# ishine/minimax-speech

Hardware: AMD Instinct MI355X
Metric: 24 kHz audio-seconds generated per wall-second per node (CosyVoice2-0.5B-shaped LM + flow + DAC-VAE, end to end) (higher is better)
Workload: dtype bf16

## Files before the change

### minimax-speech_amd/csrc/fused.hip

```cpp
#include "common.h"
#include "../../include/mmx_hip.h"
#include <type_traits>

namespace {

typedef __attribute__((ext_vector_type(4))) unsigned int u32x4_t;

__device__ unsigned long long* g_tail_stamps = nullptr;
#define TSTAMP(i) do { if constexpr (LAB) { if (st && lane == 0) st[(i)] = __builtin_amdgcn_s_memtime(); } } while (0)

template <typename T> struct FT;
template <> struct FT<bf16_t> { static constexpr int E = 8, KB = 32; typedef short8_t frag_t; };
template <> struct FT<float> { static constexpr int E = 4, KB = 16; typedef float4_t frag_t; };

template <typename T>
__device__ __forceinline__ float4_t mma(typename FT<T>::frag_t a, typename FT<T>::frag_t b, float4_t c) {
    if constexpr (sizeof(T) == 2) {
        return __builtin_amdgcn_mfma_f32_16x16x32_bf16(a, b, c, 0, 0, 0);
    } else {
#pragma unroll
        for (int s = 0; s < 4; ++s) c = __builtin_amdgcn_mfma_f32_16x16x4f32(a[s], b[s], c, 0, 0, 0);
        return c;
    }
}

__host__ __device__ constexpr int tile_pitch(int K, int esz) { return ((K * esz + 255) & ~255) + 32; }

template <typename T, int NF, int PF_>
struct WRing {
    static constexpr int E = FT<T>::E, PF = PF_;
    u32x4_t w[PF][NF];
    __device__ __forceinline__ void prime(const T* wb, long ns, int nk, int nf) {
#pragma unroll
        for (int p = 0; p < PF; ++p)
#pragma unroll
            for (int j = 0; j < NF; ++j)
                w[p][j] = *reinterpret_cast<const u32x4_t*>(wb + (j < nf ? j : 0) * ns + (long)(p < nk ? p : nk - 1) * 64 * E);
    }
};

template <typename T, int MF, int NF, int PF, int NS = 1, int RW = 4>
__device__ __forceinline__ void stage_run(WRing<T, RW, PF>& ring, const char* a_lane, int pitch, int cin_steps,
                                          const T* wb, long ns, int nk, const T* wbn, long nsn, int nkn, int nfn,
                                          float4_t (&acc)[MF][NF], int plane = 0, int tap_pitch = 0) {
    constexpr int E = FT<T>::E, KB = FT<T>::KB;
    typedef typename FT<T>::frag_t frag_t;
    if (tap_pitch == 0) tap_pitch = pitch;
    constexpr int AD = (PF % 2) ? PF : ((MF == 1 && PF >= 4) ? 4 : 2);
    static_assert(PF % AD == 0, "ring depths");
    if constexpr (NS == 2 && MF == 4) {
        frag_t a2[2][MF];
        int rt = 0, rc = 0, rs = 0, rp = 0;
        auto read_u = [&](frag_t (&dst)[MF]) {
            const char* ap = a_lane + rt * tap_pitch + rc * (KB * (int)sizeof(T)) + rp * plane;
#pragma unroll
            for (int i = 0; i < MF; ++i) dst[i] = *reinterpret_cast<const frag_t*>(ap + i * 16 * pitch);
            if (rp == 0) rp = 1;
            else {
                rp = 0;
                if (rs + 1 < nk) {
                    ++rs;
                    if (++rc == cin_steps) { rc = 0; ++rt; }
                }
            }
        };
        auto group2 = [&](int ks, auto last_c) {
            constexpr bool LAST = decltype(last_c)::value;
#pragma unroll
            for (int p = 0; p < PF; ++p) {
                frag_t b[NF];
#pragma unroll
                for (int jj = 0; jj < NF; ++jj) b[jj] = __builtin_bit_cast(frag_t, ring.w[p][jj]);
                if constexpr (LAST) {
                    if (wbn) {
                        const T* src = wbn + (long)(p < nkn ? p : nkn - 1) * 64 * E;
#pragma unroll
                        for (int jj = 0; jj < RW; ++jj) ring.w[p][jj] = *reinterpret_cast<const u32x4_t*>(src + (jj < nfn ? jj : 0) * nsn);
                    }
                } else {
                    const T* src = wb + (long)(ks + p + PF) * 64 * E;
#pragma unroll
                    for (int jj = 0; jj < NF; ++jj) ring.w[p][jj] = *reinterpret_cast<const u32x4_t*>(src + jj * ns);
                }
#pragma unroll
                for (int s2 = 0; s2 < 2; ++s2) {
                    read_u(a2[(s2 + 1) & 1]);
                    __builtin_amdgcn_sched_barrier(0);
#pragma unroll
                    for (int i = 0; i < MF; ++i)
#pragma unroll
                        for (int jj = 0; jj < NF; ++jj) acc[i][jj] = mma<T>(a2[s2][i], b[jj], acc[i][jj]);
                    __builtin_amdgcn_sched_barrier(0);
                }
            }
        };
        read_u(a2[0]);
        for (int ks = 0; ks + PF < nk; ks += PF) group2(ks, std::false_type{});
        group2(nk - PF, std::true_type{});
        return;
    }
    frag_t a[AD][NS][MF];
    int rt = 0, rc = 0, rs = 0;
    auto read_a = [&](frag_t (&dst)[NS][MF]) {
        const char* ap = a_lane + rt * tap_pitch + rc * (KB * (int)sizeof(T));
#pragma unroll
        for (int s2 = 0; s2 < NS; ++s2)
#pragma unroll
            for (int i = 0; i < MF; ++i) dst[s2][i] = *reinterpret_cast<const frag_t*>(ap + s2 * plane + i * 16 * pitch);
        if (rs + 1 < nk) {
            ++rs;
            if (++rc == cin_steps) { rc = 0; ++rt; }
        }
    };
    auto group = [&](int ks, auto last_c) {
        constexpr bool LAST = decltype(last_c)::value;
#pragma unroll
        for (int p = 0; p < PF; ++p) {
            read_a(a[(p + AD - 1) % AD]);
            frag_t b[NF];
#pragma unroll
            for (int jj = 0; jj < NF; ++jj) b[jj] = __builtin_bit_cast(frag_t, ring.w[p][jj]);
            if constexpr (LAST) {
                if (wbn) {
                    const T* src = wbn + (long)(p < nkn ? p : nkn - 1) * 64 * E;
#pragma unroll
                    for (int jj = 0; jj < RW; ++jj) ring.w[p][jj] = *reinterpret_cast<const u32x4_t*>(src + (jj < nfn ? jj : 0) * nsn);
                }
            } else {
                const T* src = wb + (long)(ks + p + PF) * 64 * E;
#pragma unroll
                for (int jj = 0; jj < NF; ++jj) ring.w[p][jj] = *reinterpret_cast<const u32x4_t*>(src + jj * ns);
            }
            __builtin_amdgcn_sched_barrier(0);
#pragma unroll
            for (int s2 = 0; s2 < NS; ++s2)
#pragma unroll
                for (int i = 0; i < MF; ++i)
#pragma unroll
                    for (int jj = 0; jj < NF; ++jj) acc[i][jj] = mma<T>(a[p % AD][s2][i], b[jj], acc[i][jj]);
            __builtin_amdgcn_sched_barrier(0);
        }
    };
#pragma unroll
    for (int s_ = 0; s_ < AD - 1; ++s_) read_a(a[s_]);
    for (int ks = 0; ks + PF < nk; ks += PF) group(ks, std::false_type{});
    group(nk - PF, std::true_type{});
}

template <typename T, int MF, int NF, int PF, int NS, int RW, bool WP>
__device__ __forceinline__ void stage_run_w(WRing<T, RW, PF>& ring, const char* a_lane, int pitch, int cin_steps,
                                            const T* wb, long ns, int nk, long wlo, const T* wbn, long nsn, int nkn, int nfn,
                                            float4_t (&acc)[MF][NF], int plane = 0, int tap_pitch = 0) {
    if constexpr (!WP) {
        stage_run<T, MF, NF, PF, NS, RW>(ring, a_lane, pitch, cin_steps, wb, ns, nk, wbn, nsn, nkn, nfn, acc, plane, tap_pitch);
    } else {
        stage_run<T, MF, NF, PF, NS, RW>(ring, a_lane, pitch, cin_steps, wb, ns, nk, wb + wlo, ns, nk, NF, acc, plane, tap_pitch);
        stage_run<T, MF, NF, PF, 1, RW>(ring, a_lane, pitch, cin_steps, wb + wlo, ns, nk, wbn, nsn, nkn, nfn, acc, 0, tap_pitch);
    }
}

template <int MF, int NF>
__device__ __forceinline__ void zero_acc(float4_t (&acc)[MF][NF]) {
#pragma unroll
    for (int i = 0; i < MF; ++i)
#pragma unroll
        for (int j = 0; j < NF; ++j) acc[i][j] = float4_t{0.f, 0.f, 0.f, 0.f};
}

constexpr int PATCH_FLOATS = 16 * 68;
constexpr int TAIL_PRM_FLOATS = 6 * 256 + 1024;
template <int NF>
__device__ __forceinline__ void to_rows(const float4_t (&acc)[NF], float* patch, int lane, float (&v)[NF * 4]) {
    constexpr int LDC = NF * 16 + 4;
    const int g = lane >> 4, l16 = lane & 15;
#pragma unroll
    for (int j = 0; j < NF; ++j)
#pragma unroll
        for (int r = 0; r < 4; ++r) patch[(4 * g + r) * LDC + j * 16 + l16] = acc[j][r];
    __builtin_amdgcn_fence(__ATOMIC_RELEASE, "wavefront");
    __builtin_amdgcn_wave_barrier();
    const float* src = patch + (lane >> 2) * LDC + (lane & 3) * (NF * 4);
#pragma unroll
    for (int c = 0; c < NF * 4; c += 4) {
        const float4_t t = *reinterpret_cast<const float4_t*>(src + c);
        v[c] = t[0]; v[c + 1] = t[1]; v[c + 2] = t[2]; v[c + 3] = t[3];
    }
    __builtin_amdgcn_wave_barrier();
}

constexpr int SPATCH_FLOATS = 16 * 20;
__device__ __forceinline__ void to_rows_sp(const float4_t (&acc)[2], float* patch, int lane, float (&v)[8]) {
    constexpr int LDC = 20;
    const int g = lane >> 4, l16 = lane & 15;
    const float* src = patch + (lane >> 2) * LDC + (lane & 1) * 8;
#pragma unroll
    for (int j = 0; j < 2; ++j) {
#pragma unroll
        for (int r = 0; r < 4; ++r) patch[(4 * g + r) * LDC + l16] = acc[j][r];
        __builtin_amdgcn_fence(__ATOMIC_RELEASE, "wavefront");
        __builtin_amdgcn_wave_barrier();
        if (((lane >> 1) & 1) == j) {
            const float4_t t0 = *reinterpret_cast<const float4_t*>(src), t1 = *reinterpret_cast<const float4_t*>(src + 4);
            v[0] = t0[0]; v[1] = t0[1]; v[2] = t0[2]; v[3] = t0[3];
            v[4] = t1[0]; v[5] = t1[1]; v[6] = t1[2]; v[7] = t1[3];
        }
        __builtin_amdgcn_wave_barrier();
    }
}
template <int NF, bool SP>
__device__ __forceinline__ void rows_of(const float4_t (&acc)[NF], float* patch, int lane, float (&v)[NF * 4]) {
// ... 495 lines not shown
        __syncthreads();
        TSTAMP(HK ? sb + 2 : 14 + ch * 12);
        const T* wn = ch + 1 < NCH ? w1_pass((ch + 1) * PPC) : (p.next.wqkv ? qkv_pass<T, NW, PW>(p.next.wqkv, wave, lane, 0) : nullptr);
        if constexpr (WP && !HK) {
            constexpr int NKQ = NK2 / 2;
            const T* wh = w2_w + (long)(ch * NK2) * 64 * E;
            stage_run_w<T, MF, NFN, PF, NS, PW, WP>(ring, buf0 + l16 * P0 + g * 16, P0, NKQ, wh, ns2, NKQ, (long)C * CF, wh + (long)NKQ * 64 * E, ns2, NKQ, NFN, acc2, PL0);
            stage_run_w<T, MF, NFN, PF, NS, PW, WP>(ring, buf0 + NKQ * KB * (int)sizeof(T) + l16 * P0 + g * 16, P0, NKQ, wh + (long)NKQ * 64 * E, ns2, NKQ, (long)C * CF, wn, ns1, NK1, PW, acc2, PL0);
        } else
        stage_run_w<T, MF, NFN, PF, NS, PW, WP>(ring, buf0 + l16 * P0 + g * 16, P0, NK2, w2_w + (long)(ch * NK2) * 64 * E, ns2, NK2, (long)C * CF, wn, ns1, NK1, PW, acc2, PL0);
        TSTAMP(HK ? sb + 3 : 15 + ch * 12);
        __syncthreads();
        TSTAMP(HK ? sb + 4 : 16 + ch * 12);
    }
    float* wpatch = HK ? reinterpret_cast<float*>(buf0) + wave * PATCH_FLOATS : patch;
    {
        float* xw = p.x + (long)b * p.x_bs;
        float b2[CW];
        loadn<CW>(prm + PRM_B2 + col0, b2);
#pragma unroll
        for (int i = 0; i < MF; ++i) {
            float v[CW];
            to_rows<NFN>(acc2[i], wpatch, lane, v);
            const int t = t0 + i * 16 + rl;
#pragma unroll
            for (int c = 0; c < CW; ++c) x1[i][c] = (x1[i][c] + v[c] + b2[c]) * rm[i];
            if (t < Tn) {
                storen<CW>(xw + (long)t * C + col0, x1[i]);
                if (p.act_out)
                    storen_T<TI, CW>(reinterpret_cast<TI*>(p.act_out) + (long)b * p.act_bs + (long)t * p.act_ld + col0, x1[i]);
            }
        }
    }
    TSTAMP(31);
    if (p.next.wqkv) {
        float n1g[CW], n1b[CW];
        loadn<CW>(prm + PRM_N1G + col0, n1g);
        loadn<CW>(prm + PRM_N1B + col0, n1b);
        ln_qkv<T, MF, PF, NW, NS, PW, WP>(x1, n1g, n1b, p.next, p.eps, a1, wpatch, stats, ring, b, t0, Tn, wave, lane, PL1, st);
    }
    TSTAMP(63);
}

template <typename T, int BM, int PF, int NW, int NS = 1, int OCC = 1, int PW = 4, bool WP = false>
__global__ __launch_bounds__(64 * NW, OCC) void est_tail_kernel(MmxEstTailParams p) {
    est_tail_tile<T, BM, PF, NW, NS, PW, WP>(p, blockIdx.x);
}

template <typename T, int BM, int PF, int NW, int NS = 1, bool WP = false>
__global__ __launch_bounds__(64 * NW) void est_resnet_kernel(MmxEstResnetParams p) {
    constexpr int MF = BM / 16, MH = MF + 1, E = FT<T>::E, KB = FT<T>::KB, C = 256;
    constexpr int WC = C / NW, CW = WC / 4, NFN = WC / 16;
    constexpr int P1 = tile_pitch(C, sizeof(T));
    constexpr int PLH = (BM + 16) * P1;
    constexpr bool PRECISE = sizeof(T) == 4;
    extern __shared__ __attribute__((aligned(16))) char smem[];
    const int cin = p.cin;
    const int PA = tile_pitch(cin, sizeof(T));
    const int PLA = (BM + 18) * PA;
    char* ain = smem;
    char* h1 = ain + NS * PLA;
    float* patch_all = reinterpret_cast<float*>(h1 + NS * PLH);
    float* stats = patch_all + NW * PATCH_FLOATS;
    const int tid = threadIdx.x, lane = tid & 63, wave = tid >> 6;
    const int g = lane >> 4, l16 = lane & 15, rl = lane >> 2;
    float* patch = patch_all + wave * PATCH_FLOATS;
    const int b = blockIdx.y, t0 = p.t_begin + blockIdx.x * BM, Tn = p.T;
    const int col0 = wave * WC + (lane & 3) * CW;
    const int cs = cin / KB;
    const T* w1 = reinterpret_cast<const T*>(p.w1) + (long)lane * E;
    const T* w2 = reinterpret_cast<const T*>(p.w2) + (long)lane * E;
    const T* wr = reinterpret_cast<const T*>(p.wr) + (long)lane * E;
    const int nk1 = 3 * cs, nk2 = 3 * (C / KB), nkr = cs;
    const long ns1 = (long)nk1 * 64 * E, ns2 = (long)nk2 * 64 * E, nsr = (long)nkr * 64 * E;
    const T* w1_w = w1 + (long)(wave * NFN) * ns1;
    const T* w2_w = w2 + (long)(wave * NFN) * ns2;
    const T* wr_w = wr + (long)(wave * NFN) * nsr;
    WRing<T, 4, PF> ring;
    ring.prime(w1_w, ns1, nk1, NFN);
    const float* rmk = p.rowmask ? p.rowmask + (long)b * p.rm_bs : nullptr;
    float bb[CW], tv[CW], gg[CW], be[CW], rm1[MH];
    loadn<CW>(p.b1 + col0, bb);
    loadn<CW>(p.tv + (long)b * p.tv_bs + col0, tv);
    loadn<CW>(p.g1 + col0, gg);
    loadn<CW>(p.be1 + col0, be);
#pragma unroll
    for (int i = 0; i < MH; ++i) {
        const int t = t0 - 16 + i * 16 + rl;
        rm1[i] = (t >= 0 && t < Tn) ? (rmk ? rmk[t] : 1.f) : 0.f;
    }
    if constexpr (NS == 1) load_tile<T>(reinterpret_cast<const T*>(p.a_in) + (long)b * p.a_bs, p.lda, t0 - 18, Tn, BM + 18, cin, ain, PA, tid, 64 * NW);
    else load_tile_split(reinterpret_cast<const float*>(p.a_in) + (long)b * p.a_bs, p.lda, t0 - 18, Tn, BM + 18, cin, ain, PA, PLA, tid, 64 * NW);
    __syncthreads();

    {
        float4_t acc[MH][NFN];
        zero_acc(acc);
        stage_run_w<T, MH, NFN, PF, NS, 4, WP>(ring, ain + l16 * PA + g * 16, PA, cs, w1_w, ns1, nk1, (long)C * 3 * cin, w2_w, ns2, nk2, NFN, acc, PLA);
        float hv[MH][CW];
#pragma unroll
        for (int i = 0; i < MH; ++i) {
            to_rows<NFN>(acc[i], patch, lane, hv[i]);
#pragma unroll
            for (int c = 0; c < CW; ++c) hv[i][c] += bb[c];
        }
        layernorm_rows<MH, CW, NW>(hv, stats, gg, be, p.eps, wave, lane);
#pragma unroll
        for (int i = 0; i < MH; ++i) {
            const int t = t0 - 16 + i * 16 + rl;
            float o[CW];
#pragma unroll
            for (int c = 0; c < CW; ++c) {
                const float y = act_c<ACT_MISH, PRECISE>(hv[i][c], 0.f) * rm1[i];
                o[c] = t >= 0 ? (y + tv[c]) * rm1[i] : 0.f;
            }
            store_tile<T, NS, CW>(h1 + (i * 16 + rl) * P1 + col0 * (int)sizeof(T), PLH, o);
        }
    }
    float br[CW];
    loadn<CW>(p.b2 + col0, bb);
    loadn<CW>(p.g2 + col0, gg);
    loadn<CW>(p.be2 + col0, be);
    loadn<CW>(p.br + col0, br);
    __syncthreads();
    float h2[MF][CW];
    {
        float4_t acc[MF][NFN];
        zero_acc(acc);
        stage_run_w<T, MF, NFN, PF, NS, 4, WP>(ring, h1 + (14 + l16) * P1 + g * 16, P1, C / KB, w2_w, ns2, nk2, (long)C * 3 * C, wr_w, nsr, nkr, NFN, acc, PLH);
#pragma unroll
        for (int i = 0; i < MF; ++i) {
            to_rows<NFN>(acc[i], patch, lane, h2[i]);
#pragma unroll
            for (int c = 0; c < CW; ++c) h2[i][c] += bb[c];
        }
        layernorm_rows<MF, CW, NW>(h2, stats, gg, be, p.eps, wave, lane);
#pragma unroll
        for (int i = 0; i < MF; ++i)
#pragma unroll
            for (int c = 0; c < CW; ++c) h2[i][c] = act_c<ACT_MISH, PRECISE>(h2[i][c], 0.f) * rm1[i + 1];
    }
    {
        if (p.next.wqkv) { loadn<CW>(p.next.n1g + col0, gg); loadn<CW>(p.next.n1b + col0, be); }
        float4_t acc[MF][NFN];
        zero_acc(acc);
        const T* wq0 = p.next.wqkv ? qkv_pass<T, NW>(p.next.wqkv, wave, lane, 0) : nullptr;
        stage_run_w<T, MF, NFN, PF, NS, 4, WP>(ring, ain + (18 + l16) * PA + g * 16, PA, cs, wr_w, nsr, nkr, (long)C * cin, wq0, (long)(C / KB) * 64 * E, C / KB, 4, acc, PLA);
        float* xw = p.x + (long)b * p.x_bs;
#pragma unroll
        for (int i = 0; i < MF; ++i) {
            float v[CW];
            to_rows<NFN>(acc[i], patch, lane, v);
            const int t = t0 + i * 16 + rl;
#pragma unroll
            for (int c = 0; c < CW; ++c) h2[i][c] += v[c] + br[c];
            if (t < Tn) storen<CW>(xw + (long)t * C + col0, h2[i]);
        }
    }
    __syncthreads();
    if (p.next.wqkv) ln_qkv<T, MF, PF, NW, NS, 4, WP>(h2, gg, be, p.next, p.eps, h1, patch, stats, ring, b, t0, Tn, wave, lane, PLH);
}


__host__ __device__ constexpr int dac_pitch(int cp) { return (((cp * 2 + 31) / 32) | 1) * 32; }
constexpr int DAC_PATCH_FLOATS = 16 * 52;

template <int C, int BM, int WR, int WC, int NS, int PF, bool WP = false>
__global__ __launch_bounds__(256) void dac_ru_kernel(MmxDacRuParams p) {
    typedef bf16_t T;
    constexpr int E = 8, KB = 32, NF = 3, CP = (C + 31) / 32 * 32, PA = dac_pitch(CP);
    constexpr int BMW = BM / WR, MF = BMW / 16;
    constexpr int NK7 = 7 * CP / KB, NK1 = CP / KB;
    constexpr bool PRECISE = NS > 1;
    static_assert(WR * WC == 4 && WC * NF * 16 == C && NK7 % PF == 0 && NK1 % PF == 0, "wave grid / ring depth");
    typedef std::conditional_t<NS == 1, bf16_t, float> TA;
    extern __shared__ __attribute__((aligned(16))) char smem[];
    const int d = p.dil, halo = 3 * d, rows_in = BM + 2 * halo;
    const int PLA = rows_in * PA, PLM = BM * PA;
    char* ain = smem;
    char* mid = ain + NS * PLA;
    float* patch_all = reinterpret_cast<float*>(mid + NS * PLM);
    float* prm = patch_all + 4 * DAC_PATCH_FLOATS;
    auto snk = [](float x, float alpha, float inv) {
        const float sn = PRECISE ? sin_cw(alpha * x) : __sinf(alpha * x);
        return x + inv * (sn * sn);
    };
    const int tid = threadIdx.x, lane = tid & 63, wave = tid >> 6;
    const int g = lane >> 4, l16 = lane & 15, rl = lane >> 2;
    const int wr = wave / WC, wc = wave % WC;
    float* patch = patch_all + wave * DAC_PATCH_FLOATS;
    const int b = blockIdx.y, t0 = blockIdx.x * BM;
    const int len = p.lens ? p.lens[b] : p.T;
    const int lc = len > 0 ? len : 1;
    const float* xb = p.x + (long)b * p.x_bs;

    const T* w7 = reinterpret_cast<const T*>(p.w7) + (long)lane * E;
    const T* w1 = reinterpret_cast<const T*>(p.w1) + (long)lane * E;
    const long ns7 = (long)NK7 * 64 * E, ns1 = (long)NK1 * 64 * E;
    const T* w7_w = w7 + (long)(wc * NF) * ns7;
    const T* w1_w = w1 + (long)(wc * NF) * ns1;
    WRing<T, NF, PF> ring;
    ring.prime(w7_w, ns7, NK7, NF);

    for (int id = tid; id < 8 * CP; id += 256) {
        const int v = id / CP, c = id - v * CP;
        const float* src = v == 0 ? p.a0 : v == 1 ? p.a2 : v == 2 ? p.b7 : v == 3 ? p.b1 : v == 4 ? p.alpha_next : v == 5 ? p.a0 : v == 6 ? p.a2 : p.alpha_next;
        const float val = (c < C && src) ? src[c] : 0.f;
        prm[id] = v < 5 ? val : 1.0f / (val + 1e-9f);
    }
    __syncthreads();
    {
        constexpr int CPR = CP / 4, U = 16;
// ... 98 lines not shown
        loadn<12>(prm + 4 * CP + col, an);
        loadn<12>(prm + 7 * CP + col, in);
        float* xo = p.x_out + (long)b * p.x_bs;
#pragma unroll
        for (int i = 0; i < MF; ++i) {
            float v[12];
            to_rows<NF>(acc[i], patch, lane, v);
            const int t = t0 + wr * BMW + i * 16 + rl;
            const bool live = t < len;
#pragma unroll
            for (int c = 0; c < 12; ++c) {
                float y = v[c] + b1[c];
                y = y > 0.f ? y : y * p.slope;
                v[c] = live ? y + xr[i][c] : 0.f;
            }
            if (t < p.T) {
                storen<12>(xo + (long)t * C + col, v);
                if (p.act_out) {
#pragma unroll
                    for (int c = 0; c < 12; ++c) v[c] = snk(v[c], an[c], in[c]);
                    TA* ao = reinterpret_cast<TA*>(p.act_out) + (long)b * p.x_bs + (long)t * C + col;
                    if constexpr (NS == 1) {
                        uint2 h0, h1, h2;
                        h0.x = pack_bf16x2(v[0], v[1]); h0.y = pack_bf16x2(v[2], v[3]);
                        h1.x = pack_bf16x2(v[4], v[5]); h1.y = pack_bf16x2(v[6], v[7]);
                        h2.x = pack_bf16x2(v[8], v[9]); h2.y = pack_bf16x2(v[10], v[11]);
                        *reinterpret_cast<uint2*>(ao) = h0;
                        *reinterpret_cast<uint2*>(ao + 4) = h1;
                        *reinterpret_cast<uint2*>(ao + 8) = h2;
                    } else {
                        storen<12>(reinterpret_cast<float*>(ao), v);
                    }
                }
            }
        }
    }
}

template <int C, int BM, int NS>
size_t dac_ru_lds(int dil) {
    constexpr int CP = (C + 31) / 32 * 32, PA = dac_pitch(CP);
    return (size_t)NS * ((size_t)(BM + 6 * dil) * PA + (size_t)BM * PA) + 4 * DAC_PATCH_FLOATS * 4 + 8 * CP * 4;
}

template <typename T, int BM, int NW, int NS = 1>
size_t tail_lds() {
    if (NS == 2 && BM == 64 && sizeof(T) == 2)
        return (size_t)NS * 2 * BM * tile_pitch(256, sizeof(T)) + (size_t)NW * SPATCH_FLOATS * 4 + (size_t)BM * NW * 4 + (size_t)TAIL_PRM_FLOATS * 4;
    return NS * ((size_t)BM * tile_pitch(512, sizeof(T)) + (size_t)BM * tile_pitch(256, sizeof(T))) + (size_t)NW * PATCH_FLOATS * 4 + (size_t)BM * NW * 4 +
           (size_t)TAIL_PRM_FLOATS * 4;
}
template <typename T, int BM, int NW, int NS = 1>
size_t resnet_lds(int cin) {
    return NS * ((size_t)(BM + 18) * tile_pitch(cin, sizeof(T)) + (size_t)(BM + 16) * tile_pitch(256, sizeof(T))) + (size_t)NW * PATCH_FLOATS * 4 +
           (size_t)(BM + 16) * NW * 4;
}

int check_next(const MmxEstNext& nx, int dtype, int T_) {
    if (!nx.wqkv) return MMX_OK;
    MMX_CHECK_ARG(nx.n1g && nx.n1b && nx.q_out);
    MMX_CHECK_ARG(((uintptr_t)nx.q_out % 16) == 0 && nx.q_bs % 8 == 0);
    if (dtype == MMX_X2) {
        if (nx.vt_out) {
            MMX_CHECK_ARG(nx.ldq % 8 == 0 && nx.ldq >= 2048 && nx.q_bs % 8 == 0 && nx.ldvt % 8 == 0 && nx.ldvt >= ((T_ + 7) / 8) * 8);
            MMX_CHECK_ARG(((uintptr_t)nx.vt_out % 16) == 0 && nx.vt_bs % 8 == 0 && nx.vt_bs >= 2 * 512 * (int64_t)nx.ldvt);
        } else {
            MMX_CHECK_ARG(nx.ldq % 4 == 0 && nx.ldq >= 1536 && nx.q_bs % 4 == 0);
        }
    } else if (dtype == MMX_BF16) {
        MMX_CHECK_ARG(nx.vt_out && nx.ldq % 8 == 0 && nx.ldq >= 1024 && nx.ldvt % 8 == 0 && nx.ldvt >= ((T_ + 7) / 8) * 8);
        MMX_CHECK_ARG(((uintptr_t)nx.vt_out % 16) == 0 && nx.vt_bs % 8 == 0);
    } else {
        MMX_CHECK_ARG(nx.ldq % 4 == 0 && nx.ldq >= 1536);
    }
    return MMX_OK;
}

}

#if MMX_LAB
extern "C" int mmx_lab_tail_stamps(void* buf) {
    unsigned long long* p = reinterpret_cast<unsigned long long*>(buf);
    const hipError_t e = hipMemcpyToSymbol(HIP_SYMBOL(g_tail_stamps), &p, sizeof(p));
    return e == hipSuccess ? MMX_OK : -(int)e - 1000;
}
#endif

extern "C" int mmx_est_tail(const MmxEstTailParams* pp, int dtype, int bm, int cfg, hipStream_t stream) {
    MMX_CHECK_ARG(pp != nullptr);
    const MmxEstTailParams& p = *pp;
    const bool wplanes = dtype == MMX_X2W;
    if (wplanes) dtype = MMX_X2;
    MMX_CHECK_ARG(p.ao && p.x && p.wo && p.w1 && p.w2 && p.bo && p.b1 && p.b2 && p.n3g && p.n3b && p.B > 0 && p.T > 0);
    MMX_CHECK_ARG(p.t_begin >= 0 && p.t_begin < p.T && p.t_begin % 16 == 0);
    MMX_CHECK_ARG(p.ldao >= 512 && p.ldao % (dtype == MMX_X2 ? 4 : 8) == 0 && p.ao_bs % (dtype == MMX_X2 ? 4 : 8) == 0 && p.x_bs % 4 == 0);
    MMX_CHECK_ARG(((uintptr_t)p.ao % 16) == 0 && ((uintptr_t)p.x % 16) == 0);
    MMX_CHECK_ARG(!p.act_out || (p.act_ld % (dtype == MMX_X2 ? 4 : 8) == 0 && p.act_bs % (dtype == MMX_X2 ? 4 : 8) == 0 && ((uintptr_t)p.act_out % 16) == 0));
    if (int rc = check_next(p.next, dtype, p.T)) return rc;
    const int nw = (cfg >> 4) & 15, occ2 = (cfg >> 8) & 1;
#define TAILT(TT, BM, PF, NW, NS, OCC, PW, ...)                                                           \
    do {                                                                                                   \
        const size_t lds = tail_lds<TT, BM, NW, NS>();                                                     \
        MMX_CHECK_ARG(lds * OCC <= 160 * 1024);                                                            \
        MMX_LDS_OPT_IN((est_tail_kernel<TT, BM, PF, NW, NS, OCC, PW __VA_OPT__(,) __VA_ARGS__>), lds);     \
        hipLaunchKernelGGL((est_tail_kernel<TT, BM, PF, NW, NS, OCC, PW __VA_OPT__(,) __VA_ARGS__>), dim3((p.T - p.t_begin + BM - 1) / BM, p.B), dim3(64 * NW), lds, stream, p); \
    } while (0)
// ... 40 lines not shown
        } else return MMX_EARG;
    } else if (dtype == MMX_F32) {
        if (bm == 32 && (nw == 0 || nw == 4)) TAIL(float, 32, 4, 4);
        else if (bm == 16 && (nw == 0 || nw == 4)) TAIL(float, 16, 8, 4);
        else return MMX_EARG;
    } else return MMX_EARG;
#undef TAIL
#undef TAILN
#undef TAILO
#undef TAILP
#undef TAILT
    MMX_LAUNCH_CHECK();
    return MMX_OK;
}

extern "C" int mmx_est_resnet(const MmxEstResnetParams* pp, int dtype, int bm, int cfg, hipStream_t stream) {
    MMX_CHECK_ARG(pp != nullptr);
    const MmxEstResnetParams& p = *pp;
    const bool wplanes = dtype == MMX_X2W;
    if (wplanes) dtype = MMX_X2;
    MMX_CHECK_ARG(p.a_in && p.x && p.w1 && p.w2 && p.wr && p.b1 && p.b2 && p.br && p.g1 && p.be1 && p.g2 && p.be2 && p.tv);
    MMX_CHECK_ARG(p.t_begin >= 0 && p.t_begin < p.T && p.t_begin % 16 == 0);
    MMX_CHECK_ARG(p.B > 0 && p.T > 0 && p.cin >= 64 && p.cin % 32 == 0 && p.cin <= 512 && p.lda >= p.cin);
    MMX_CHECK_ARG(p.lda % (dtype == MMX_X2 ? 4 : 8) == 0 && p.a_bs % (dtype == MMX_X2 ? 4 : 8) == 0);
    MMX_CHECK_ARG(((uintptr_t)p.a_in % 16) == 0 && ((uintptr_t)p.x % 16) == 0 && p.x_bs % 4 == 0 && p.tv_bs % 4 == 0 && ((uintptr_t)p.tv % 16) == 0);
    if (int rc = check_next(p.next, dtype, p.T)) return rc;
    const int pf_req = cfg & 15, nw = cfg >> 4;
#define RESNN(TT, BM, PF, NW, NS, ...)                                                                    \
    do {                                                                                                   \
        const size_t lds = resnet_lds<TT, BM, NW, NS>(p.cin);                                              \
        MMX_CHECK_ARG(lds <= 160 * 1024);                                                                  \
        MMX_LDS_OPT_IN((est_resnet_kernel<TT, BM, PF, NW, NS __VA_OPT__(,) __VA_ARGS__>), lds);            \
        hipLaunchKernelGGL((est_resnet_kernel<TT, BM, PF, NW, NS __VA_OPT__(,) __VA_ARGS__>), dim3((p.T - p.t_begin + BM - 1) / BM, p.B), dim3(64 * NW), lds, stream, p); \
    } while (0)
#define RESN(TT, BM, PF, NW) RESNN(TT, BM, PF, NW, 1)
    const int kb = dtype == MMX_F32 ? 16 : 32;
    if (dtype == MMX_X2) {
        int pfx = pf_req > 0 ? pf_req : 4;
        while (pfx > 2 && ((3 * p.cin / kb) % pfx || (p.cin / kb) % pfx || (256 / kb) % pfx)) pfx /= 2;
        MMX_CHECK_ARG((p.cin / kb) % 2 == 0);
        if (bm == 32) {
            MMX_CHECK_ARG((resnet_lds<bf16_t, 32, 4, 2>(p.cin)) <= 160 * 1024);
            if (wplanes && nw != 4 && (resnet_lds<bf16_t, 32, 8, 2>(p.cin)) <= 160 * 1024) { if (pfx >= 4) RESNN(bf16_t, 32, 4, 8, 2, true); else RESNN(bf16_t, 32, 2, 8, 2, true); }
            else if (wplanes) { if (pfx >= 4) RESNN(bf16_t, 32, 4, 4, 2, true); else RESNN(bf16_t, 32, 2, 4, 2, true); }
            else if (nw != 4 && (resnet_lds<bf16_t, 32, 8, 2>(p.cin)) <= 160 * 1024) { if (pfx >= 4) RESNN(bf16_t, 32, 4, 8, 2); else RESNN(bf16_t, 32, 2, 8, 2); }
            else if (pfx >= 4) RESNN(bf16_t, 32, 4, 4, 2); else RESNN(bf16_t, 32, 2, 4, 2);
        } else if (bm == 16) {
            if (nw != 4 && (resnet_lds<bf16_t, 32, 8, 2>(p.cin)) <= 160 * 1024) {
                if (wplanes) { if (pfx >= 4) RESNN(bf16_t, 16, 4, 8, 2, true); else RESNN(bf16_t, 16, 2, 8, 2, true); }
                else if (pfx >= 4) RESNN(bf16_t, 16, 4, 8, 2); else RESNN(bf16_t, 16, 2, 8, 2);
            }
            else if (wplanes) { if (pfx >= 4) RESNN(bf16_t, 16, 4, 4, 2, true); else RESNN(bf16_t, 16, 2, 4, 2, true); }
            else if (pfx >= 4) RESNN(bf16_t, 16, 4, 4, 2); else RESNN(bf16_t, 16, 2, 4, 2);
        } else return MMX_EARG;
        MMX_LAUNCH_CHECK();
        return MMX_OK;
    }
    const size_t lds8 = bm == 64 ? resnet_lds<bf16_t, 64, 8>(p.cin) : (bm == 32 ? resnet_lds<bf16_t, 32, 8>(p.cin) : resnet_lds<bf16_t, 16, 8>(p.cin));
    const bool w8 = dtype == MMX_BF16 && (nw == 8 || (nw == 0 && lds8 <= 160 * 1024));
    const int want = pf_req > 0 ? pf_req : (w8 ? (bm == 64 ? 2 : 4) : (bm == 16 ? 8 : 4));
    MMX_CHECK_ARG(want == 2 || want == 4 || want == 8);
    int pf = want;
    while (pf > 2 && ((3 * p.cin / kb) % pf || (p.cin / kb) % pf || (256 / kb) % pf)) pf /= 2;
    MMX_CHECK_ARG((p.cin / kb) % 2 == 0 && (nw == 0 || nw == 4 || nw == 8));
    if (dtype == MMX_BF16) {
        if (w8) {
            if (bm == 64) RESN(bf16_t, 64, 2, 8);
            else if (bm == 32) { if (pf >= 4) RESN(bf16_t, 32, 4, 8); else RESN(bf16_t, 32, 2, 8); }
            else if (bm == 16) { if (pf >= 4) RESN(bf16_t, 16, 4, 8); else RESN(bf16_t, 16, 2, 8); }
            else return MMX_EARG;
        } else {
            if (bm == 64) { if (pf >= 4) RESN(bf16_t, 64, 4, 4); else RESN(bf16_t, 64, 2, 4); }
            else if (bm == 32) { if (pf >= 4) RESN(bf16_t, 32, 4, 4); else RESN(bf16_t, 32, 2, 4); }
            else if (bm == 16) { if (pf == 8) RESN(bf16_t, 16, 8, 4); else if (pf == 4) RESN(bf16_t, 16, 4, 4); else RESN(bf16_t, 16, 2, 4); }
            else return MMX_EARG;
        }
    } else if (dtype == MMX_F32) {
        if (bm == 16 && (nw == 0 || nw == 4)) { if (pf == 8) RESN(float, 16, 8, 4); else if (pf == 4) RESN(float, 16, 4, 4); else RESN(float, 16, 2, 4); }
        else return MMX_EARG;
    } else return MMX_EARG;
#undef RESN
#undef RESNN
    MMX_LAUNCH_CHECK();
    return MMX_OK;
}

extern "C" int mmx_dac_ru(const MmxDacRuParams* pp, int dtype, int bm, hipStream_t stream) {
    MMX_CHECK_ARG(pp != nullptr);
    const MmxDacRuParams& p = *pp;
    MMX_CHECK_ARG(p.x && p.x_out && p.x != p.x_out && p.w7 && p.w1 && p.b7 && p.b1 && p.a0 && p.a2 && p.B > 0 && p.T > 0);
    MMX_CHECK_ARG(p.dil >= 1 && p.dil <= 9 && (p.C == 48 || p.C == 96 || p.C == 192) && p.x_bs % 4 == 0 && p.x_bs >= (int64_t)p.T * p.C);
    MMX_CHECK_ARG(((uintptr_t)p.x % 16) == 0 && ((uintptr_t)p.x_out % 16) == 0 && ((uintptr_t)p.act_out % 16) == 0 && ((uintptr_t)p.a0 % 16) == 0);
    MMX_CHECK_ARG(!p.act_out || p.alpha_next);
    const bool wplanes = dtype == MMX_X2W;
    if (wplanes) dtype = MMX_X2;
    MMX_CHECK_ARG(dtype == MMX_BF16 || dtype == MMX_X2);
#define DACRU(C_, BM_, WR_, WC_, NS_, PF_, ...)                                                            \
    do {                                                                                                   \
        const size_t lds = dac_ru_lds<C_, BM_, NS_>(p.dil);                                                \
        MMX_CHECK_ARG(lds <= 160 * 1024);                                                                  \
        MMX_LDS_OPT_IN((dac_ru_kernel<C_, BM_, WR_, WC_, NS_, PF_ __VA_OPT__(,) __VA_ARGS__>), lds);       \
        hipLaunchKernelGGL((dac_ru_kernel<C_, BM_, WR_, WC_, NS_, PF_ __VA_OPT__(,) __VA_ARGS__>), dim3((p.T + BM_ - 1) / BM_, p.B), dim3(256), lds, stream, p); \
    } while (0)
    if (wplanes) {
        if (bm != 0 && bm != (p.C == 48 ? 64 : p.C == 96 ? (p.dil > 3 ? 128 : 64) : 32)) return MMX_EARG;
        if (p.C == 48) DACRU(48, 64, 4, 1, 2, 2, true);
// ... 19 lines not shown
```

### minimax-speech_amd/mmx/flow.py

```python
import gc
import itertools
import math
from collections import OrderedDict
from typing import Dict, Optional

import torch

from . import ops
from ._lib import BF16, F32, TORCH_DT, WEIGHT_DT, X2, X2W, is_split


def espnet_rel_pe(T: int, d: int) -> torch.Tensor:
    pos = torch.arange(T - 1, -T, -1, dtype=torch.float32)[:, None]
    div = torch.exp(torch.arange(0, d, 2, dtype=torch.float32) * -(math.log(10000.0) / d))
    pe = torch.zeros(2 * T - 1, d)
    pe[:, 0::2] = torch.sin(pos * div)
    pe[:, 1::2] = torch.cos(pos * div)
    return pe


import threading

CAPTURE_LOCK = threading.RLock()

# ... 483 lines not shown
        self._walk(stage, S, B, T, mask)
        return S["d"]

    def _walk(self, stage, S, B, T, mask=None, r0=0, Tc=None):
        dt, C, Tc = self.dtype, self.C, Tc or T
        assert mask is None or r0 == 0

        def conv3(src, ld, w, b, rowmask, out_act=None, out_f32=None):
            N = w.shape[0]
            ops.gemm(src, w, T - r0, N, dtype=dt, lda=ld, cin=C, ntaps=3, row_off=r0 - 2, row_lo=0, row_hi=T, batch=B,
                     a_bstride=Tc * ld, bias=b, rowmask=rowmask, rm_bstride=Tc, out_act=(None if out_act is None else out_act[:, r0:]),
                     ldo_a=N, oa_bstride=Tc * N, out_f32=(None if out_f32 is None else out_f32[:, r0:]), ldo_f=N, of_bstride=Tc * N)

        stage(self.down, S["h0"], 320, S["cat"][:, :, C:], 2 * C)
        conv3(S["cat"][:, :, C:], 2 * C, self.down_w, self.down_b, mask, out_act=S["amid"][0])
        for i, sw in enumerate(self.mid):
            last = i == len(self.mid) - 1
            stage(sw, S["amid"][i], C, S["cat"] if last else S["amid"][i + 1], 2 * C if last else C)
        stage(self.up, S["cat"], 2 * C, S["aup"], C)
        conv3(S["aup"], C, self.up_w, self.up_b, mask, out_act=S["a2"])
        conv3(S["a2"], C, self.fin_w, self.fin_b, None, out_f32=S["c1"])
        ops.rownorm(S["c1"][:, r0:], self.fin_g, self.fin_be, 1e-5, rows=T - r0, C_=C, batch=B, x_bstride=Tc * C, act="mish",
                    rowmask=mask, out_act=S["afin"][:, r0:], o_bstride=Tc * C, dtype=dt)
        ops.gemm(S["afin"][:, r0:], self.proj_w, T - r0, 80, dtype=dt, lda=C, cin=C, row_hi=T - r0, batch=B, a_bstride=Tc * C,
                 bias=self.proj_b, rowmask=mask, rm_bstride=Tc, out_f32=S["d"][:, r0:], ldo_f=80, of_bstride=Tc * 80)

    _WG_US = {16: 27.1, 32: 29.9, 64: 44.1}
    _WG_US_X = {16: 29.1, 32: 35.8, 64: 60.3}
    _WG_US_XW = {16: 46.9, 32: 52.6, 64: 81.2}

    @classmethod
    def _launch_us(cls, bm, tiles, split=False):
        wg = (cls._WG_US_XW if split == "w" else cls._WG_US_X if split else cls._WG_US)[bm]
        t = lambda n: wg * (1.0 + 0.45 * (n / 256.0) ** 2)
        full, rem = divmod(tiles, 256)
        return full * t(256) + (t(rem) if rem else 0.0)

    def _tile_rows(self, B, T):
        tiles = lambda bm: B * ((T + bm - 1) // bm)
        if self.dtype == BF16:
            cap = getattr(self, "max_tile_rows", 64)
            bm = min((b for b in (64, 32, 16) if b <= cap), key=lambda b: (self._launch_us(b, tiles(b)), -b))
            bm = max(bm, getattr(self, "min_tile_rows", 16), 64 if self.polite else 16)
            return bm, bm
        if self.split:
            cap = getattr(self, "max_tile_rows", 64)
            bm = min((b for b in (64, 32, 16) if b <= cap), key=lambda b: (self._launch_us(b, tiles(b), "w" if self.wplanes else True), -b))
            if self.polite:
                bm = max(bm, min(cap, 64))
            br = 32 if (tiles(32) >= 128 or self.polite) else 16
            return bm, br
        return (32 if tiles(32) >= 128 else 16), 16

    def _estimator_rows(self, S, tv, B, T, chunk, attn_bufs, mask=None, klen=None, r0=0, Tc=None, fp8=False, form=0):
        dt, C, Tc = self.dtype, self.C, Tc or T
        bm_t, bm_r = self._tile_rows(B, T - r0)
        ntv = tv.shape[1]

        def nxt(w, qk, vt):
            return ops.est_next(wqkv=w["wqkv_p"], n1g=w["n1g"], n1b=w["n1b"], q_out=qk, ldq=qk.shape[-1], q_bs=Tc * qk.shape[-1],
                                vt_out=vt, ldvt=(0 if vt is None else vt.shape[-1]), vt_bs=(0 if vt is None else vt[0].numel()))

        def stage(sw, a_in, lda, act_out, act_ld):
            r, blocks = sw["res"], sw["blocks"]
            bufs = [next(attn_bufs) for _ in blocks]
            ops.est_resnet(a_in, lda, lda, S["xs"], r, tv[:, r["idx"] * C:], ntv, B=B, T=T, dtype=dt,
                           bm=(16 if (self.split and lda > 320) else bm_r), rowmask=mask, nxt=nxt(blocks[0], *bufs[0]),
                           t_begin=r0, Tcap=Tc)
            for j, w in enumerate(blocks):
                last = j == len(blocks) - 1
                self._attention(*bufs[j], S["ao"], B=B, T=T, chunk=chunk, mask=mask, klen=klen, q_begin=r0, fp8=fp8, form=form)
                ops.est_tail(S["ao"], S["xs"], w, B=B, T=T, dtype=dt, bm=bm_t, rowmask=(mask if last else None),
                             act_out=(act_out if last else None), act_ld=act_ld,
                             nxt=(None if last else nxt(blocks[j + 1], *bufs[j + 1])), t_begin=r0, Tcap=Tc)

        self._walk(stage, S, B, T, mask, r0, Tc)

    class StreamState:

        def __init__(self, eng, Tcap):
            self.eng, self.Tcap, self.T = eng, ops.round_up(Tcap, 64), 0
            self.steps = [None] * eng.n_timesteps
            self.lat = torch.zeros(self.Tcap, 80, device=eng.dev)
            Tc, new = self.Tcap, eng._new
            self.xs, self.c1 = new(2, Tc, eng.C, f32=True), new(2, Tc, eng.C, f32=True)
            self.ao, self.afin, self.d = new(2, Tc, 512), new(2, Tc, eng.C), new(2, Tc, 80, f32=True)
            tt, dd = eng.t_schedule()
            self.t_all = torch.tensor([[v, v] for v in tt], dtype=torch.float32, device=eng.dev)
            self.dt = dd
            self.enc = None
            self.tok_done = 0
            self.z = eng.rand_noise[0, :, :self.Tcap].t().contiguous().to(eng.dev)
            self.cond = torch.zeros(self.Tcap, 80, device=eng.dev)
            self.spks2 = torch.zeros(2, 80, device=eng.dev)
            self.ids = torch.zeros(self.Tcap // 2 + eng.L + 8, dtype=torch.int64, device=eng.dev)
            self.graphs, self._win = {}, {}
            self.busy = False

        def release(self):
            for g in self.graphs.values():
                g.release()
            self.graphs, self._win, self.steps, self.enc = {}, {}, [None] * self.eng.n_timesteps, None

        def window(self, n):
            if n not in self._win:
                d = self.eng.dev
                self._win[n] = dict(x=torch.zeros(1, n, 80, device=d), mu2=torch.zeros(2, n, 80, device=d),
                                    cond2=torch.zeros(2, n, 80, device=d))
            return self._win[n]

        def reset(self):
            self.T = self.tok_done = 0

        def step_buffers(self, s):
            if self.steps[s] is None:
                e, Tc = self.eng, self.Tcap
                z = lambda *sh, dtype=e.tdt: torch.zeros(*sh, dtype=dtype, device=e.dev)
                nblk = 4 * (2 + len(e.mid))
                ldq, qdt, planes = e._attn_layout(presplit=False)
                self.steps[s] = dict(h0=z(2, Tc, 320), amid=[z(2, Tc, e.C) for _ in e.mid], cat=z(2, Tc, 2 * e.C), aup=z(2, Tc, e.C),
# ... 252 lines not shown
```

Baseline: 560.9.

## Add 64-row split-bf16 resnet tile with trimmed halo and reused patch LDS

```diff
diff --git a/minimax-speech_amd/csrc/fused.hip b/minimax-speech_amd/csrc/fused.hip
--- a/minimax-speech_amd/csrc/fused.hip
+++ b/minimax-speech_amd/csrc/fused.hip
@@ -39,22 +39,23 @@
     }
 };
 
-template <typename T, int MF, int NF, int PF, int NS = 1, int RW = 4>
+template <typename T, int MF, int NF, int PF, int NS = 1, int RW = 4, bool H0 = false>
 __device__ __forceinline__ void stage_run(WRing<T, RW, PF>& ring, const char* a_lane, int pitch, int cin_steps,
                                           const T* wb, long ns, int nk, const T* wbn, long nsn, int nkn, int nfn,
-                                          float4_t (&acc)[MF][NF], int plane = 0, int tap_pitch = 0) {
+                                          float4_t (&acc)[MF][NF], int plane = 0, int tap_pitch = 0, int d0 = 0) {
     constexpr int E = FT<T>::E, KB = FT<T>::KB;
     typedef typename FT<T>::frag_t frag_t;
     if (tap_pitch == 0) tap_pitch = pitch;
+    auto frag_off = [&](int i) { return H0 ? (i == 0 ? d0 : (i - 1) * 16 * pitch) : i * 16 * pitch; };
     constexpr int AD = (PF % 2) ? PF : ((MF == 1 && PF >= 4) ? 4 : 2);
     static_assert(PF % AD == 0, "ring depths");
-    if constexpr (NS == 2 && MF == 4) {
+    if constexpr (NS == 2 && (MF == 4 || H0)) {
         frag_t a2[2][MF];
         int rt = 0, rc = 0, rs = 0, rp = 0;
         auto read_u = [&](frag_t (&dst)[MF]) {
             const char* ap = a_lane + rt * tap_pitch + rc * (KB * (int)sizeof(T)) + rp * plane;
 #pragma unroll
-            for (int i = 0; i < MF; ++i) dst[i] = *reinterpret_cast<const frag_t*>(ap + i * 16 * pitch);
+            for (int i = 0; i < MF; ++i) dst[i] = *reinterpret_cast<const frag_t*>(ap + frag_off(i));
             if (rp == 0) rp = 1;
             else {
                 rp = 0;
@@ -106,7 +107,7 @@
 #pragma unroll
         for (int s2 = 0; s2 < NS; ++s2)
 #pragma unroll
-            for (int i = 0; i < MF; ++i) dst[s2][i] = *reinterpret_cast<const frag_t*>(ap + s2 * plane + i * 16 * pitch);
+            for (int i = 0; i < MF; ++i) dst[s2][i] = *reinterpret_cast<const frag_t*>(ap + s2 * plane + frag_off(i));
         if (rs + 1 < nk) {
             ++rs;
             if (++rc == cin_steps) { rc = 0; ++rt; }
@@ -147,15 +148,15 @@
     group(nk - PF, std::true_type{});
 }
 
-template <typename T, int MF, int NF, int PF, int NS, int RW, bool WP>
+template <typename T, int MF, int NF, int PF, int NS, int RW, bool WP, bool H0 = false>
 __device__ __forceinline__ void stage_run_w(WRing<T, RW, PF>& ring, const char* a_lane, int pitch, int cin_steps,
                                             const T* wb, long ns, int nk, long wlo, const T* wbn, long nsn, int nkn, int nfn,
-                                            float4_t (&acc)[MF][NF], int plane = 0, int tap_pitch = 0) {
+                                            float4_t (&acc)[MF][NF], int plane = 0, int tap_pitch = 0, int d0 = 0) {
     if constexpr (!WP) {
-        stage_run<T, MF, NF, PF, NS, RW>(ring, a_lane, pitch, cin_steps, wb, ns, nk, wbn, nsn, nkn, nfn, acc, plane, tap_pitch);
+        stage_run<T, MF, NF, PF, NS, RW, H0>(ring, a_lane, pitch, cin_steps, wb, ns, nk, wbn, nsn, nkn, nfn, acc, plane, tap_pitch, d0);
     } else {
-        stage_run<T, MF, NF, PF, NS, RW>(ring, a_lane, pitch, cin_steps, wb, ns, nk, wb + wlo, ns, nk, NF, acc, plane, tap_pitch);
-        stage_run<T, MF, NF, PF, 1, RW>(ring, a_lane, pitch, cin_steps, wb + wlo, ns, nk, wbn, nsn, nkn, nfn, acc, 0, tap_pitch);
+        stage_run<T, MF, NF, PF, NS, RW, H0>(ring, a_lane, pitch, cin_steps, wb, ns, nk, wb + wlo, ns, nk, NF, acc, plane, tap_pitch, d0);
+        stage_run<T, MF, NF, PF, 1, RW, H0>(ring, a_lane, pitch, cin_steps, wb + wlo, ns, nk, wbn, nsn, nkn, nfn, acc, 0, tap_pitch, d0);
     }
 }
 
@@ -757,19 +758,23 @@
     constexpr int MF = BM / 16, MH = MF + 1, E = FT<T>::E, KB = FT<T>::KB, C = 256;
     constexpr int WC = C / NW, CW = WC / 4, NFN = WC / 16;
     constexpr int P1 = tile_pitch(C, sizeof(T));
-    constexpr int PLH = (BM + 16) * P1;
+    constexpr bool TRIM = NS == 2 && BM == 64 && sizeof(T) == 2;
+    static_assert(!TRIM || NW == 8, "64-row split tile: 8 waves (one-fragment patches serve 32-column slices)");
+    constexpr int HA = TRIM ? 4 : 18, HH = TRIM ? 2 : 16;
+    constexpr int PLH = (BM + HH) * P1;
     constexpr bool PRECISE = sizeof(T) == 4;
     extern __shared__ __attribute__((aligned(16))) char smem[];
     const int cin = p.cin;
     const int PA = tile_pitch(cin, sizeof(T));
-    const int PLA = (BM + 18) * PA;
+    const int PLA = (BM + HA) * PA;
     char* ain = smem;
     char* h1 = ain + NS * PLA;
     float* patch_all = reinterpret_cast<float*>(h1 + NS * PLH);
-    float* stats = patch_all + NW * PATCH_FLOATS;
+    constexpr int PATCHF = TRIM ? SPATCH_FLOATS : PATCH_FLOATS;
+    float* stats = patch_all + NW * PATCHF;
     const int tid = threadIdx.x, lane = tid & 63, wave = tid >> 6;
     const int g = lane >> 4, l16 = lane & 15, rl = lane >> 2;
-    float* patch = patch_all + wave * PATCH_FLOATS;
+    float* patch = patch_all + wave * PATCHF;
     const int b = blockIdx.y, t0 = p.t_begin + blockIdx.x * BM, Tn = p.T;
     const int col0 = wave * WC + (lane & 3) * CW;
     const int cs = cin / KB;
@@ -794,18 +799,22 @@
         const int t = t0 - 16 + i * 16 + rl;
         rm1[i] = (t >= 0 && t < Tn) ? (rmk ? rmk[t] : 1.f) : 0.f;
     }
-    if constexpr (NS == 1) load_tile<T>(reinterpret_cast<const T*>(p.a_in) + (long)b * p.a_bs, p.lda, t0 - 18, Tn, BM + 18, cin, ain, PA, tid, 64 * NW);
-    else load_tile_split(reinterpret_cast<const float*>(p.a_in) + (long)b * p.a_bs, p.lda, t0 - 18, Tn, BM + 18, cin, ain, PA, PLA, tid, 64 * NW);
+    if constexpr (NS == 1) load_tile<T>(reinterpret_cast<const T*>(p.a_in) + (long)b * p.a_bs, p.lda, t0 - HA, Tn, BM + HA, cin, ain, PA, tid, 64 * NW);
+    else load_tile_split(reinterpret_cast<const float*>(p.a_in) + (long)b * p.a_bs, p.lda, t0 - HA, Tn, BM + HA, cin, ain, PA, PLA, tid, 64 * NW);
     __syncthreads();
 
     {
         float4_t acc[MH][NFN];
         zero_acc(acc);
+        if constexpr (TRIM) {
+            const int d0 = ((l16 > 14 ? l16 - 14 : 0) - (l16 + 2)) * PA;
+            stage_run_w<T, MH, NFN, PF, NS, 4, WP, true>(ring, ain + (l16 + 2) * PA + g * 16, PA, cs, w1_w, ns1, nk1, (long)C * 3 * cin, w2_w, ns2, nk2, NFN, acc, PLA, 0, d0);
+        } else
         stage_run_w<T, MH, NFN, PF, NS, 4, WP>(ring, ain + l16 * PA + g * 16, PA, cs, w1_w, ns1, nk1, (long)C * 3 * cin, w2_w, ns2, nk2, NFN, acc, PLA);
         float hv[MH][CW];
 #pragma unroll
         for (int i = 0; i < MH; ++i) {
-            to_rows<NFN>(acc[i], patch, lane, hv[i]);
+            rows_of<NFN, TRIM>(acc[i], patch, lane, hv[i]);
 #pragma unroll
             for (int c = 0; c < CW; ++c) hv[i][c] += bb[c];
         }
@@ -819,6 +828,9 @@
                 const float y = act_c<ACT_MISH, PRECISE>(hv[i][c], 0.f) * rm1[i];
                 o[c] = t >= 0 ? (y + tv[c]) * rm1[i] : 0.f;
             }
+            if constexpr (TRIM) {
+                if (i > 0 || rl >= 14) store_tile<T, NS, CW>(h1 + (i * 16 + rl - 14) * P1 + col0 * (int)sizeof(T), PLH, o);
+            } else
             store_tile<T, NS, CW>(h1 + (i * 16 + rl) * P1 + col0 * (int)sizeof(T), PLH, o);
         }
     }
@@ -832,10 +844,10 @@
     {
         float4_t acc[MF][NFN];
         zero_acc(acc);
-        stage_run_w<T, MF, NFN, PF, NS, 4, WP>(ring, h1 + (14 + l16) * P1 + g * 16, P1, C / KB, w2_w, ns2, nk2, (long)C * 3 * C, wr_w, nsr, nkr, NFN, acc, PLH);
+        stage_run_w<T, MF, NFN, PF, NS, 4, WP>(ring, h1 + (HH - 2 + l16) * P1 + g * 16, P1, C / KB, w2_w, ns2, nk2, (long)C * 3 * C, wr_w, nsr, nkr, NFN, acc, PLH);
 #pragma unroll
         for (int i = 0; i < MF; ++i) {
-            to_rows<NFN>(acc[i], patch, lane, h2[i]);
+            rows_of<NFN, TRIM>(acc[i], patch, lane, h2[i]);
 #pragma unroll
             for (int c = 0; c < CW; ++c) h2[i][c] += bb[c];
         }
@@ -850,7 +862,11 @@
         float4_t acc[MF][NFN];
         zero_acc(acc);
         const T* wq0 = p.next.wqkv ? qkv_pass<T, NW>(p.next.wqkv, wave, lane, 0) : nullptr;
-        stage_run_w<T, MF, NFN, PF, NS, 4, WP>(ring, ain + (18 + l16) * PA + g * 16, PA, cs, wr_w, nsr, nkr, (long)C * cin, wq0, (long)(C / KB) * 64 * E, C / KB, 4, acc, PLA);
+        stage_run_w<T, MF, NFN, PF, NS, 4, WP>(ring, ain + (HA + l16) * PA + g * 16, PA, cs, wr_w, nsr, nkr, (long)C * cin, wq0, (long)(C / KB) * 64 * E, C / KB, 4, acc, PLA);
+        if constexpr (TRIM) {
+            __syncthreads();
+            patch = reinterpret_cast<float*>(ain) + wave * PATCH_FLOATS;
+        }
         float* xw = p.x + (long)b * p.x_bs;
 #pragma unroll
         for (int i = 0; i < MF; ++i) {
@@ -862,7 +878,7 @@
             if (t < Tn) storen<CW>(xw + (long)t * C + col0, h2[i]);
         }
     }
-    __syncthreads();
+    if constexpr (!TRIM) __syncthreads();
     if (p.next.wqkv) ln_qkv<T, MF, PF, NW, NS, 4, WP>(h2, gg, be, p.next, p.eps, h1, patch, stats, ring, b, t0, Tn, wave, lane, PLH);
 }
 
@@ -1067,6 +1083,9 @@
 }
 template <typename T, int BM, int NW, int NS = 1>
 size_t resnet_lds(int cin) {
+    if (NS == 2 && BM == 64 && sizeof(T) == 2)
+        return NS * ((size_t)(BM + 4) * tile_pitch(cin, sizeof(T)) + (size_t)(BM + 2) * tile_pitch(256, sizeof(T))) + (size_t)NW * SPATCH_FLOATS * 4 +
+               (size_t)(BM + 16) * NW * 4;
     return NS * ((size_t)(BM + 18) * tile_pitch(cin, sizeof(T)) + (size_t)(BM + 16) * tile_pitch(256, sizeof(T))) + (size_t)NW * PATCH_FLOATS * 4 +
            (size_t)(BM + 16) * NW * 4;
 }
@@ -1213,6 +1232,10 @@
             }
             else if (wplanes) { if (pfx >= 4) RESNN(bf16_t, 16, 4, 4, 2, true); else RESNN(bf16_t, 16, 2, 4, 2, true); }
             else if (pfx >= 4) RESNN(bf16_t, 16, 4, 4, 2); else RESNN(bf16_t, 16, 2, 4, 2);
+        } else if (bm == 64) {
+            MMX_CHECK_ARG(nw != 4 && (resnet_lds<bf16_t, 64, 8, 2>(p.cin)) <= 160 * 1024);
+            if (wplanes) RESNN(bf16_t, 64, 2, 8, 2, true);
+            else if (pf_req >= 4 && pfx >= 4) RESNN(bf16_t, 64, 4, 8, 2); else RESNN(bf16_t, 64, 2, 8, 2);
         } else return MMX_EARG;
         MMX_LAUNCH_CHECK();
         return MMX_OK;
diff --git a/minimax-speech_amd/mmx/flow.py b/minimax-speech_amd/mmx/flow.py
--- a/minimax-speech_amd/mmx/flow.py
+++ b/minimax-speech_amd/mmx/flow.py
@@ -559,6 +559,19 @@
             return bm, br
         return (32 if tiles(32) >= 128 else 16), 16
 
+    resnet64_polite = True
+
+    def _resnet_rows(self, bm_r, lda, B, T):
+        if not self.split:
+            return bm_r
+        if lda > 320:
+            return 16
+        if lda > 256:
+            return min(bm_r, 32)
+        if getattr(self, "max_tile_rows", 64) >= 64 and (B * ((T + 31) // 32) > 256 or (self.polite and self.resnet64_polite)):
+            return 64
+        return bm_r
+
     def _estimator_rows(self, S, tv, B, T, chunk, attn_bufs, mask=None, klen=None, r0=0, Tc=None, fp8=False, form=0):
         dt, C, Tc = self.dtype, self.C, Tc or T
         bm_t, bm_r = self._tile_rows(B, T - r0)
@@ -572,7 +585,7 @@
             r, blocks = sw["res"], sw["blocks"]
             bufs = [next(attn_bufs) for _ in blocks]
             ops.est_resnet(a_in, lda, lda, S["xs"], r, tv[:, r["idx"] * C:], ntv, B=B, T=T, dtype=dt,
-                           bm=(16 if (self.split and lda > 320) else bm_r), rowmask=mask, nxt=nxt(blocks[0], *bufs[0]),
+                           bm=self._resnet_rows(bm_r, lda, B, T - r0), rowmask=mask, nxt=nxt(blocks[0], *bufs[0]),
                            t_begin=r0, Tcap=Tc)
             for j, w in enumerate(blocks):
                 last = j == len(blocks) - 1
```

Result: no change. 564.5, median of 6 (+0.6%).
